# cvxgrp/qcqp

Measured on AMD Instinct MI355X. Metric: restarts x coord-sweeps / sec (improve COORD_DESCENT phase-2 sweeps, 2n^2 flops each; whole step timed), higher is better.
Workload: dtype f64

## Files before the change

### qcqp_amd/csrc/capi_stream.hip

```cpp
#include <chrono>
#include <cstdio>
#include <cstdlib>

#include "capi_ctx.h"
#include "cd_life.h"

using namespace qcqpmi;

namespace {

StreamShape stream_shape(const qcqpmi_ctx *c) {
    StreamShape s;
    s.NB = (int)(c->n16 / 16); s.sep = c->sep; s.maxc = c->maxc; s.Kreal = c->Kreal; s.objclass = c->objclass; s.symcls = c->symcls;
    s.queue_ok = cd_queue_shape_ok(c);
    return s;
}

StreamSwitches stream_switches(const qcqpmi_ctx *c) {
    StreamSwitches s;
    s.life_version = c->life_version; s.force_generic = c->force_generic; s.dbg = c->dbg; s.lr_RB = c->lr_RB; s.profile = c->profile;
    const char *ev = getenv("QCQPMI_L2_PREBUILT");
    s.prebuilt = !(ev && atoi(ev) == 0);
    ev = getenv("QCQPMI_L2_Y0_MAX");
    s.y0_max = ev ? atoll(ev) : STREAM_Y0_ALL;
    ev = getenv("QCQPMI_L2_ROT");
    s.rot = ev ? atoi(ev) : STREAM_ROT_AUTO;
    ev = getenv("QCQPMI_L2_TILES");
    s.tiles = ev ? atoi(ev) : 0;
    return s;
}

int stream_plan_for(qcqpmi_ctx *c, int64_t K, int64_t R, StreamPlan *P) {
    int cus = 0;
    HIPCHK(c, hipDeviceGetAttribute(&cus, hipDeviceAttributeMultiprocessorCount, c->device));
    *P = stream_plan(stream_shape(c), stream_switches(c), K, R, cus);
    return 0;
}

int cd_bestK_reserve(qcqpmi_ctx *c, size_t K) {
    HIPCHK(c, c->d_bestK_idx.reserve(c->stream, K * 2, false));
    HIPCHK(c, c->d_bestK_key.reserve(c->stream, K * 2, false));
    HIPCHK(c, c->d_bestK_x.reserve(c->stream, K * (size_t)c->n, false));
    return 0;
}

int cd_life2_reserve(qcqpmi_ctx *c, size_t scratch) {
    HIPCHK(c, c->l2_scratch.reserve(c->stream, scratch));
    HIPCHK(c, c->l2_abort.reserve(c->stream, 4));
    HIPCHK(c, c->l2_cuslot.reserve(c->stream, 4096));
    if (!c->l2_S) {
        const size_t NB = (size_t)(c->n16 / 16);
        HIPCHK(c, c->l2_D.reserve(c->stream, NB * 256));
        HIPCHK(c, c->l2_S.reserve(c->stream, NB * 48));
        hipError_t e = (hipError_t)cd_life2_pack(c->dp, c->l2_D, c->l2_S, c->stream);
        if (e != hipSuccess) return fail(c, QCQPMI_EHIP, "cd_life2_pack: %s", hipGetErrorString(e));
    }
    return 0;
}

int cd_life2_pre_reserve(qcqpmi_ctx *c, const StreamPlan &P) {
    HIPCHK(c, c->l2_preslack.reserve(c->stream, P.l2_preslack));
    HIPCHK(c, c->l2_y0.reserve(c->stream, P.l2_y0, false));
    return 0;
}

int stream_reserve(qcqpmi_ctx *c, const StreamPlan &P, bool winners) {
    int rc;
    if (P.outputs && (rc = cd_outputs_reserve(c, (int64_t)P.outputs))) return rc;
    if (winners && P.bestK && (rc = cd_bestK_reserve(c, P.bestK))) return rc;
    HIPCHK(c, c->d_qnext.reserve(c->stream, 16));
    HIPCHK(c, c->d_life.reserve(c->stream, 1, false));
    if (P.kernel == STREAM_LIFE2 && (rc = cd_life2_reserve(c, P.l2_scratch))) return rc;
    if (P.pre && (rc = cd_life2_pre_reserve(c, P))) return rc;
    return 0;
}

struct StreamClock {
    const bool on = getenv("QCQPMI_STREAM_TIMING") != nullptr;
    double stage[6] = {0, 0, 0, 0, 0, 0}, step[6] = {0, 0, 0, 0, 0, 0};
    static double now() { return std::chrono::duration<double, std::milli>(std::chrono::steady_clock::now().time_since_epoch()).count(); }
    void at_stage(int k) { stage[k] = now(); }
    void at_step(int k) { step[k] = now(); }
    void report_launch() const {
        if (on) fprintf(stderr, "cd_stream_run launch (ms): reserve %.3f, event %.3f, launch call %.3f, event + spin wait %.3f, copy call %.3f, sync %.3f\n", step[0] - stage[1], step[1] - step[0], step[2] - step[1], step[3] - step[2], step[4] - step[3], step[5] - step[4]);
    }
    void report() const {
        if (on) fprintf(stderr, "cd_stream_run timing (ms): set-up %.3f, launch + kernel %.3f, fetch %.3f, status %.3f, best %.3f\n", stage[1] - stage[0], stage[2] - stage[1],
                        stage[3] - stage[2], stage[4] - stage[3], stage[5] - stage[4]);
    }
};

struct StreamRun {
    int64_t K, R, num_iters;
    double tol;
    uint64_t seed, first_index;
};

int stream_fill_life(qcqpmi_ctx *c, const StreamPlan &P, const StreamRun &r, int generate, int phase1, double viol_tol, uint64_t seed_stride,
                     uint64_t first_stride) {
    HIPCHK(c, hipMemsetAsync(c->d_qnext, 0, 16 * sizeof(int), c->stream));
    CdLife L;
    L.on = 1; L.generate = generate ? 1 : 0; L.phase1 = phase1 ? 1 : 0; L.Rtotal = r.K * r.R; L.Rpop = r.R;
    L.seed = r.seed; L.seed_stride = seed_stride; L.first_index = r.first_index; L.first_stride = first_stride; L.viol_tol = viol_tol;
    L.sweeps1 = c->d_sweeps1; L.status1 = c->d_status1; L.ran2 = c->d_flag;
    L.prof = nullptr;
    L.prebuilt = P.pre ? 1 : 0; L.preslack = P.pre ? (const double *)c->l2_preslack : nullptr;
    L.y0_count = P.y0_count; L.y0 = P.pre ? (const double *)c->l2_y0 : nullptr;
    if (P.life_prof) {
        HIPCHK(c, c->d_life_prof.reserve(c->stream, P.life_prof, false));
        HIPCHK(c, hipMemsetAsync(c->d_life_prof, 0, P.life_prof * sizeof(long long), c->stream));
        L.prof = c->d_life_prof;
    }
    HIPCHK(c, hipMemcpyAsync(c->d_life, &L, sizeof(L), hipMemcpyHostToDevice, c->stream));
    HIPCHK(c, spin_sync(c->stream));
    return 0;
}

int stream_launch_life2(qcqpmi_ctx *c, const StreamPlan &P, const StreamRun &r, StreamClock &clk) {
    CdLife2Args qa;
    qa.P = c->dp; qa.num_iters = r.num_iters; qa.tol = r.tol; qa.life = c->d_life;
    cd_queue_fill_batch(c, qa.b, r.seed, r.first_index);
    qa.b.R = r.K * r.R;
    qa.scratch = c->l2_scratch; qa.Dpack = c->l2_D; qa.Spack = c->l2_S; qa.abort = c->l2_abort; qa.fbound = c->fbound;
    qa.cuslot = P.rot ? (int *)c->l2_cuslot : nullptr; qa.rotmode = P.rot;
    if (qa.cuslot) HIPCHK(c, hipMemsetAsync(c->l2_cuslot, 0, 4096 * sizeof(int), c->stream));
    qa.dbg = (c->dbg & 2048) ? 1 : 0;
    qa.Gpack = P.lr ? (const double *)c->lr_G : nullptr; qa.Upack = P.lr ? (const double *)c->lr_U : nullptr; qa.RB = P.lr ? c->lr_RB : 0;
    qa.nclass = c->Kreal;
    clk.at_step(0);
    (void)hipEventRecord(c->timers[2].beg, c->stream);
    clk.at_step(1);
    hipError_t qe = P.pre ? (hipError_t)cd_life2_prep_launch(c->dp, c->d_life, c->X, r.K * r.R, r.num_iters, r.tol, c->stream) : hipSuccess;
    if (qe == hipSuccess && P.y0_count > 0)
        qe = (hipError_t)cd_life2_y0_launch(c->X, c->lr_U, c->l2_y0, (int)(c->n16 / 16), P.factor_rb, c->n16, P.y0_count, c->stream);
    if (qe == hipSuccess) qe = (hipError_t)cd_life2_launch(qa, P.nmw, P.cs, P.kind, P.tiles, (int)P.wgs, c->stream);
    clk.at_step(2);
    (void)hipEventRecord(c->timers[2].end, c->stream);
    c->timers[2].valid = true;
    if (qe != hipSuccess) return fail(c, QCQPMI_EHIP, "cd_stream_run: %s", hipGetErrorString(qe));
    c->last_cd2_kernel = P.name;
    int ab = 0;
    HIPCHK(c, spin_sync(c->stream));
    clk.at_step(3);
    HIPCHK(c, hipMemcpyAsync(&ab, c->l2_abort, sizeof(int), hipMemcpyDeviceToHost, c->stream));
    clk.at_step(4);
    HIPCHK(c, spin_sync(c->stream));
    clk.at_step(5);
    clk.report_launch();
    if (ab) {
        HIPCHK(c, hipMemsetAsync(c->l2_abort, 0, sizeof(int), c->stream));
        c->R = 0;
        return fail(c, QCQPMI_EHIP, "cd_stream_run: a wait inside cd_life_kernel ran into its watchdog (internal error; no results)");
    }
    return 0;
}

int stream_launch_round4(qcqpmi_ctx *c, const StreamPlan &P, const StreamRun &r) {
    CdQueueArgs qa;
    qa.P = c->dp; qa.num_iters = r.num_iters; qa.tol = r.tol;
    qa.life = c->d_life; qa.life_on = 1;
// ... 134 lines not shown
```

### qcqp_amd/csrc/cd_life.hip

```cpp
#include "cd_life.h"

#include <cstdio>
#include <cstdlib>

#include "onevar.h"
#include "cd_phase1_sep.h"
#include "cd_chain.h"
#include "cd_roles.h"

namespace qcqpmi {
namespace {

constexpr int L2_WD = 1 << 21;
enum { L2_ABORT = 3 };

__device__ __attribute__((always_inline)) inline RqOwn l2_own(int NB, int CS, int m, int NMW) {
    RqOwn o;
    const int rest = NB - CS;
    o.NB = NB;
    if (m < 0) { o.first = rest; o.stride = 1; o.nu = CS; }
    else { o.first = m; o.stride = NMW; o.nu = m < rest ? (rest - m + NMW - 1) / NMW : 0; }
    return o;
}

// ... 11 lines not shown
    int *p1cols = (int *)(smem + 16); \
    int *jn = (int *)(smem + 32); \
    double *sp = smem + L2_SHARED_DOUBLES + (tile_) * l2_tile_doubles(NMW, CSU, LRV, KCLV, MAXC); \
    double *part2 = sp; sp += 2 * NMW * 256; \
    double *fixp = sp; sp += 256; \
    double *gtile = sp; sp += 256; \
    double *DU2 = sp; sp += 2 * 256; \
    double *sc2 = sp; sp += 2 * 48; \
    double *ring = sp; sp += 4 * 256; \
    double *cshare = sp; sp += CSU * 256; \
    double *slk = sp; sp += 16; \
    rq_lds_int *sy = (rq_lds_int *)(int *)sp; sp += 8; \
    double *of0 = sp; sp += 16; \
    long long *ovis = (long long *)sp; sp += 16; \
    long long *oacc = (long long *)sp; sp += 16; \
    long long *oswp = (long long *)sp; sp += 16; \
    int *sid = (int *)sp; sp += 8; \
    int *snew = (int *)sp; sp += 8; \
    int *sfin = (int *)sp; sp += 8; \
    int *ost = (int *)sp; sp += 8; \
    int *gatep = (int *)sp; sp += 8; \
    long long *cst = (long long *)sp; sp += 64 * 10; \
    unsigned long long *sseed = (unsigned long long *)sp; sp += 16; \
    unsigned long long *sfirst = (unsigned long long *)sp; sp += 16; \
    unsigned long long *p1key = (unsigned long long *)sp; sp += 16; \
    int *p1upd = (int *)sp; sp += 8; \
    int *p1fin = (int *)sp; sp += 8; \
    int *p1sw = (int *)sp; sp += 8; \
    int *p1st = (int *)sp; sp += 8; \
    L2Par *par = (L2Par *)sp; sp += 32;       \
    double *ytile = sp; sp += LRV ? L2_YBMAX * 256 : 0; \
    double *pend = sp; sp += LRV ? 2 * 256 : 0; \
    SetTable<MAXC> TC;        \
    TC.slots = 16 * KCLV; \
    TC.lo = sp; sp += (MAXC + 1) * 16 * KCLV; \
    TC.hi = sp; sp += (MAXC + 1) * 16 * KCLV; \
    TC.n = (int *)sp; sp += 8 * KCLV; \
    TC.slow = (int *)sp; sp += 8 * KCLV; \
    int *clsb = (int *)sp;
template <class T>
__device__ __attribute__((always_inline)) inline T *l2_tl(T *p, int t, int tile_doubles) { return (T *)((double *)p + t * tile_doubles); }

struct L2Par {
    const double *Apack, *Apack2, *Dpack, *Spack;
    const double *Gpack, *Upack;
    int RB, pad_;
    double *Xg;
    int *next;
    unsigned long long *prof;
    long long num_iters, n16;
    double tol, r0, fbound;
    int NB, KS, n, nlast, Rtotal, dbg;
    const int *cls;
};
static_assert(sizeof(L2Par) <= 32 * sizeof(double), "L2Par outgrew its LDS slot");
struct L2Life {
    int64_t Rtotal, Rpop, y0_count;
    uint64_t seed, seed_stride, first_index, first_stride;
    const double *preslack, *y0;
    int64_t *sweeps1;
    int *status1;
    uint8_t *ran2;
    unsigned long long *prof;
    double cp, cq, cr;
    int rel, prebuilt;
    int turn, pad_;
};
static_assert(sizeof(L2Life) <= 256, "L2Life outgrew the tail of the LDS allocation");
__device__ __attribute__((always_inline)) inline int l2_uni(int v) { return __builtin_amdgcn_readfirstlane(v); }
__device__ __attribute__((always_inline)) inline long long l2_uni(long long v) {
    const int lo = __builtin_amdgcn_readfirstlane((int)(v & 0xffffffffll)), hi = __builtin_amdgcn_readfirstlane((int)(v >> 32));
    return ((long long)hi << 32) | (long long)(unsigned)lo;
}
__device__ __attribute__((always_inline)) inline double l2_uni(double v) { return __longlong_as_double(l2_uni(__double_as_longlong(v))); }
template <class T>
__device__ __attribute__((always_inline)) inline T *l2_uni(T *p) { return (T *)(uintptr_t)l2_uni((long long)(uintptr_t)p); }

template <int NMW, int CS>
__device__ __attribute__((noinline)) void l2_mfma_role(int m_in, int t_in) {
    constexpr int MAXC = 1;
    constexpr int KCLV = 1;
    constexpr int CSU = CS > 0 ? CS : 1;
    constexpr int LRV = 0;
    const int tile = l2_uni(t_in);
    L2_LDS_VIEW(tile)
    (void)ytile; (void)pend; (void)clsb;
    (void)fixp; (void)gtile; (void)DU2; (void)sc2; (void)cshare; (void)slk; (void)TC; (void)of0; (void)ovis; (void)oacc; (void)oswp; (void)sid; (void)snew;
    (void)sfin; (void)ost; (void)ctl; (void)cst; (void)sseed; (void)sfirst; (void)p1key; (void)p1upd; (void)p1fin; (void)p1sw; (void)p1st; (void)gatep; (void)simdof; (void)p1cols; (void)jn;
    const int lane = threadIdx.x & 63;
    const int m = l2_uni(m_in);
    const double *pApack2 = l2_uni(par->Apack2);
    double *pXg = l2_uni(par->Xg);
    unsigned long long *pprof = l2_uni(par->prof);
    const int NB = l2_uni(par->NB), KS = l2_uni(par->KS);
    const int64_t n16 = l2_uni(par->n16);
    const int rowmask = (l2_uni(par->dbg) & 1) ? 7 : -1;
    const int64_t gmax = (int64_t)1 << 40;
    const RqOwn own = l2_own(NB, CS, m, NMW);
    const int nu = own.nu;
    v2d_ arP[2 * RQ_PFU];
    const unsigned vlane = (unsigned)lane * 16u;
    const __amdgpu_buffer_rsrc_t arsrc = __builtin_amdgcn_make_buffer_rsrc(const_cast<double *>(pApack2), 0, NB * KS * 512, 0x00020000);
    const __amdgpu_buffer_rsrc_t xrsrc = __builtin_amdgcn_make_buffer_rsrc(pXg, 0, (int)(n16 * 128), 0x00020000);
    const int rowstride = KS * 512;
    typedef unsigned rq_u4 __attribute__((ext_vector_type(4)));
    typedef unsigned rq_u2 __attribute__((ext_vector_type(2)));
    #define L2_LDA(dst, soff, vo) { const rq_u4 t0_ = __builtin_amdgcn_raw_buffer_load_b128(arsrc, (vo), (soff), 0);           \
                            const rq_u4 t1_ = __builtin_amdgcn_raw_buffer_load_b128(arsrc, (vo) + 1024u, (soff), 0);   \
                            (dst)[0] = __builtin_bit_cast(v2d_, t0_); (dst)[1] = __builtin_bit_cast(v2d_, t1_); }
    double bq[4 * RQ_PERS];
    {
        const unsigned vl8 = (unsigned)lane * 8u;
    #pragma unroll
        for (int u = 0; u < RQ_PERS; u++)
    #pragma unroll
            for (int q = 0; q < 4; q++) {
                const rq_u2 t_ = __builtin_amdgcn_raw_buffer_load_b64(xrsrc, vl8, (m + NMW * u) * 2048 + q * 512, 0);
                bq[4 * u + q] = __builtin_bit_cast(double, t_);
            }
// ... 184 lines not shown
            for (;;) {
                const rq_i4 s4 = rq_sync_read(sy);
                if (s4[RQ_STOP]) { stop = true; break; }
                if (s4[RQ_CONS] >= (int)i - 1) break;
                if (++spins > L2_WD) { stop = true; rq_sync_write(sy, L2_ABORT, 1, lane); rq_sync_write(sy, RQ_STOP, 1, lane); break; }
                __builtin_amdgcn_s_sleep(1);
            }
            if (stop) break;
            spins = 0;
        }
        {
            double *part = part2 + (int)(i & 1) * NMW * 256 + m * 256;
    #pragma unroll
            for (int v = 0; v < 4; v++) part[v * 64 + (lane & 15) * 4 + (lane >> 4)] = acc[v];
        }
        rq_sync_write(sy, RQ_PARTS + m, (int)i + 1, lane);
        row = row2;
    }
    if (yrow == NB - 1 && iy >= 3) {
        v2d_ aU[YU][2];
    #pragma unroll
        for (int u = 0; u < YU; u++)
            if (u < nu) L2_LDF(aU[u], ursrc, ((NB - 3) * RB + m + NMW * u) * 2048)
        rq_lds_cd *src = rbase + (int)((iy - 2) & 3) * 256;
        double bd[4];
    #pragma unroll
        for (int q = 0; q < 4; q++) bd[q] = src[q * 64];
    #pragma unroll
        for (int v = 0; v < 4; v++)
    #pragma unroll
            for (int u = 0; u < YU; u++)
                if (u < nu) y[u] = __builtin_amdgcn_mfma_f64_16x16x4f64(aU[u][v >> 1][v & 1], bd[v], y[u], 0, 0, 0);
        save_y();
    } else if (yrow == 0) {
        save_y();
    }
    #undef L2_LDF
}

template <int NMW, int CS, int KIND, int TILES, int LR>
__device__ __attribute__((noinline)) void l2_chain_role(int t_in) {
    constexpr bool MULTI = KIND == L2_KIND_GENK || KIND == L2_KIND_LINK;
    constexpr int BK = KIND == L2_KIND_GENK ? L2_KIND_GEN : KIND == L2_KIND_LINK ? L2_KIND_LIN : KIND;
    constexpr int MAXC = MULTI ? 2 : 1;
    constexpr int KCLV = MULTI ? L2_KCL : 1;
    constexpr int CSU = CS > 0 ? CS : 1;
    constexpr int LRV = LR;
    static_assert(!LR || CS == 0, "factored objective: the chain has no share of the contraction");
    static_assert(!MULTI || (TILES == 1 && !LR), "multi-class kinds: one tile per workgroup, no objective factor");
    constexpr bool PRE = BK == L2_KIND_LIN || BK == L2_KIND_SGN;
    const int tile = TILES > 1 ? l2_uni(t_in) : 0;
    L2_LDS_VIEW(tile)
    (void)ytile; (void)pend; (void)clsb;
    (void)slk; (void)snew; (void)p1key; (void)p1upd; (void)p1fin; (void)p1sw; (void)p1st; (void)gatep; (void)simdof; (void)p1cols; (void)jn;
    const int lane = threadIdx.x & 63, r = lane >> 2, gq = lane & 3;
    GLB const double *Apk = glb(l2_uni(par->Apack));
    GLB const double *Apk2 = glb(l2_uni(par->Apack2));
    GLB const double *Dpk = glb(l2_uni(par->Dpack));
    GLB const double *Spk = glb(l2_uni(par->Spack));
    GLB double *Xg = glb(l2_uni(par->Xg));
    GLB const int *pnext = glb(l2_uni(par->next));
    GLB const int *clsg = glb(l2_uni(par->cls));
    unsigned long long *pprof = l2_uni(par->prof);
    const int pRtotal = l2_uni(par->Rtotal);
    const int NB = l2_uni(par->NB), KS = l2_uni(par->KS), nlast = l2_uni(par->nlast);
    struct { int64_t n; double r0; } P = {(int64_t)l2_uni(par->n), l2_uni(par->r0)};
    struct { double tol, fbound; int64_t num_iters; } a = {l2_uni(par->tol), l2_uni(par->fbound), (int64_t)l2_uni(par->num_iters)};
    const int64_t gmax = (int64_t)1 << 40;
    __builtin_amdgcn_s_setprio(3);
    const int Un = TC.n[r], Uslow = TC.slow[r];
    const double Ul0 = TC.lo[r], Uh0 = TC.hi[r], Ul1 = TC.lo[16 + r], Uh1 = TC.hi[16 + r];
    const bool two = Un >= 2;
    const double thr = two ? 1e-7 * (Ul1 - Uh0) : 0.0;
    const double syma = two ? Ul1 : 0.0, symb = two ? Uh1 : Uh0;
    const double gmid = two ? 0.5 * (Uh0 + Ul1) : QM_INF;
    const double linL = Ul0, linH = two ? Uh1 : Uh0;
    auto lin_tl = [&](double l0_, double h0_, double l1_, double h1_, bool two_) {
        const double lL = l0_, lH = two_ ? h1_ : h0_;
        const double w0 = h0_ - l0_, w1 = two_ ? h1_ - l1_ : w0;
        const double wmin = w0 < w1 ? w0 : w1;
        const double hh = fabs(lL) > fabs(lH) ? fabs(lL) : fabs(lH);
        const double scale = a.fbound * (hh * hh > 1.0 ? hh * hh : 1.0);
        return (wmin > 0.0) ? 0.5e-12 * scale / wmin : QM_INF;
    };
    double tl = 0.0;
    if ((BK == L2_KIND_LIN || BK == L2_KIND_SGN) && !MULTI) tl = lin_tl(Ul0, Uh0, Ul1, Uh1, two);
    const double omid = (BK == L2_KIND_SGN) ? 0.5 * (linL + linH) : 0.0;
    struct { int upd_counter, visits, accepted, sweeps, status; bool conv; } S;
    S.upd_counter = (int)cst[0 * 64 + lane]; S.visits = (int)cst[1 * 64 + lane]; S.accepted = (int)cst[2 * 64 + lane];
    S.sweeps = (int)cst[3 * 64 + lane]; S.conv = cst[4 * 64 + lane] != 0; S.status = (int)cst[5 * 64 + lane];
    double fpart = __longlong_as_double(cst[6 * 64 + lane]);
    bool frz = (cst[7 * 64 + lane] & 1) != 0, done = (cst[7 * 64 + lane] & 2) != 0, pre = PRE && (cst[7 * 64 + lane] & 4) != 0;
    bool ld = LR && (cst[7 * 64 + lane] & 8) != 0;
    double facc = __longlong_as_double(cst[8 * 64 + lane]);
    const bool occupied = sid[r] >= 0;
    const RqOwn cown = l2_own(NB, CS, -1, NMW);
    v2d_ arC[2 * CSU];
    double afix[4] = {0.0, 0.0, 0.0, 0.0}, afix2[4] = {0.0, 0.0, 0.0, 0.0};
    v4d_ carry = {0.0, 0.0, 0.0, 0.0};
    double xon[4], d4[4], s3 = 0.0;
    {
    #pragma unroll
        for (int e = 0; e < 4; e++) d4[e] = Dpk[lane + 64 * e];
        if (lane < 48) s3 = Spk[lane];
    #pragma unroll
        for (int v = 0; v < 4; v++) xon[v] = Xg[(4 * v + gq) * 16 + r];
    #pragma unroll
        for (int e = 0; e < 4; e++) DU2[lane + 64 * e] = d4[e];
        if (lane < 48) sc2[lane] = s3;
        if (MULTI && lane < 16) clsb[lane] = (lane < l2_uni(par->n)) ? clsg[lane] : 0;
        v4d_ c0 = {0.0, 0.0, 0.0, 0.0}, c1 = {0.0, 0.0, 0.0, 0.0};
        const int bl2 = NB - 2, bl1 = NB - 1;
        double f0a[4], f0b[4], f1b[4], x2[4], x1[4];
    #pragma unroll
        for (int u = 0; u < 4; u++) {
            f0a[u] = Apk[((int64_t)0 * KS + 4 * bl2 + u) * 64 + lane];
            f0b[u] = Apk[((int64_t)0 * KS + 4 * bl1 + u) * 64 + lane];
            f1b[u] = Apk[((int64_t)1 * KS + 4 * bl1 + u) * 64 + lane];
            x2[u] = LR ? pend[u * 64 + lane] : Xg[(4 * bl2 + u) * 64 + lane];
            x1[u] = LR ? pend[256 + u * 64 + lane] : Xg[(4 * bl1 + u) * 64 + lane];
        }
    #pragma unroll
        for (int u = 0; u < 4; u++) c0 = __builtin_amdgcn_mfma_f64_16x16x4f64(f0a[u], x2[u], c0, 0, 0, 0);
    #pragma unroll
        for (int u = 0; u < 4; u++) {
            c0 = __builtin_amdgcn_mfma_f64_16x16x4f64(f0b[u], x1[u], c0, 0, 0, 0);
            c1 = __builtin_amdgcn_mfma_f64_16x16x4f64(f1b[u], x1[u], c1, 0, 0, 0);
        }
        carry = c1;
        if (CS > 0) {
            rq_load_A<CSU>(arC, Apk2, KS, cown, lane, 0);
            double bqC[4 * CSU];
    #pragma unroll
            for (int U = 0; U < CSU; U++) {
                const int bb = rq_block(cown, U);
    #pragma unroll
                for (int q = 0; q < 4; q++) bqC[4 * U + q] = Xg[(4 * bb + q) * 64 + lane];
            }
    #pragma unroll
            for (int U = 0; U < CSU; U++)
    #pragma unroll
                for (int q = 0; q < 4; q++) cshare[U * 256 + q * 64 + lane] = bqC[4 * U + q];
            c0 = rq_product<CSU>(arC, bqC, Apk2, KS, cown, lane, rq_slot(cown, bl1), rq_slot(cown, bl2), 1, c0);
        }
    #pragma unroll
        for (int v = 0; v < 4; v++) fixp[v * 64 + (lane & 15) * 4 + (lane >> 4)] = c0[v];
    }
    const double tolv = a.tol;
    int b = 0, spins = 0;
    bool wdog = false;
    const bool prof_on = pprof != nullptr;
    long long pw_part = 0, pt_sum = 0, pt_steps = 0, pt_end = 0, pt_fix = 0, pt_req = 0, ptl = 0;
    if (prof_on) { ptl = (long long)__builtin_amdgcn_s_memtime(); if (lane == 0) atomicAdd(pprof + 18, (unsigned long long)(ptl - *(long long *)(ctl + 6))); }
    int pn_int = 0, pn_gen = 0;
#define L2_TICK(acc) if (prof_on) { const long long now_ = (long long)__builtin_amdgcn_s_memtime(); acc += now_ - ptl; ptl = now_; }
    int64_t last_g = 0;
    for (int64_t g = 0; g < gmax; g++) {
        last_g = g;
        const int bn = (b + 1 == NB) ? 0 : b + 1, bn2 = (bn + 1 == NB) ? 0 : bn + 1;
        const int bprev = (b == 0) ? NB - 1 : b - 1;
        const int cur = (int)(g & 1);
        const double *DU = DU2 + cur * 256, *hqb = sc2 + cur * 48, *rtb = sc2 + cur * 48 + 16, *dgb = sc2 + cur * 48 + 32;
        const double *part = part2 + cur * NMW * 256;
        double *rb = ring + (int)(g & 3) * 256;
        const int ncol = (b == NB - 1) ? nlast : 16;
        double xo[4];
    #pragma unroll
        for (int v = 0; v < 4; v++) xo[v] = xon[v];
    #pragma unroll
        for (int e = 0; e < 4; e++) d4[e] = Dpk[(int64_t)bn * 256 + lane + 64 * e];
        if (lane < 48) s3 = Spk[(int64_t)bn * 48 + lane];
        int c3 = 0;
        if (MULTI && lane < 16) c3 = (16 * bn + lane < (int)P.n) ? clsg[16 * bn + lane] : 0;
    #pragma unroll
        for (int v = 0; v < 4; v++) xon[v] = Xg[(16 * (int64_t)bn + 4 * v + gq) * 16 + r];
        {
            GLB const double *ap = Apk + ((int64_t)bn * KS + 4 * b) * 64 + lane;
            GLB const double *ap2 = Apk + ((int64_t)bn2 * KS + 4 * b) * 64 + lane;
    #pragma unroll
            for (int u = 0; u < 4; u++) { afix[u] = ap[u * 64]; afix2[u] = ap2[u * 64]; }
        }
        const long long tw0 = prof_on ? (long long)__builtin_amdgcn_s_memtime() : 0;
        for (;;) {
            const rq_i4 p4 = rq_sync_read(sy + RQ_PARTS);
            int lo4 = p4[0] < p4[1] ? p4[0] : p4[1];
            const int lo2 = p4[2] < p4[3] ? p4[2] : p4[3];
            lo4 = lo4 < lo2 ? lo4 : lo2;
            if (NMW > 4) {
                const rq_i4 q4 = rq_sync_read(sy + RQ_PARTS + 4);
                const int l1 = q4[0] < q4[1] ? q4[0] : q4[1], l2 = q4[2] < q4[3] ? q4[2] : q4[3];
                lo4 = lo4 < l1 ? lo4 : l1;
                lo4 = lo4 < l2 ? lo4 : l2;
            }
            if (lo4 >= (int)g + 1) break;
            if (++spins > L2_WD) { wdog = true; break; }
            __builtin_amdgcn_s_sleep(1);
        }
        if (wdog) { rq_sync_write(sy, L2_ABORT, 1, lane); break; }
        spins = 0;
        if (prof_on) { pt_req += tw0 - ptl; ptl = (long long)__builtin_amdgcn_s_memtime(); pw_part += ptl - tw0; pn_int++; }
        double gb[4], xn[4], rto[4], t2o[4], hq4[4];
    #pragma unroll
        for (int v = 0; v < 4; v++) {
            double s = fixp[v * 64 + lane];
    #pragma unroll
            for (int w = 0; w < NMW; w++) s += part[w * 256 + v * 64 + lane];
            hq4[v] = hqb[4 * v + gq];
            s += hq4[v];
            gb[v] = s;
            gtile[(4 * v + gq) * 16 + r] = s;
        }
        rq_sync_write(sy, RQ_CONS, (int)g + 1, lane);
    #pragma unroll
        for (int v = 0; v < 4; v++) { rto[v] = rtb[4 * v + gq]; t2o[v] = dgb[4 * v + gq]; }
        if (b == 0 && !S.conv && S.sweeps >= (int)a.num_iters) {
            S.conv = true;
            frz = true; facc = 0.0;
        }
        if (b == 0 && !S.conv) S.sweeps++;
        const bool act = !S.conv;
        int nv[4], slv[4];
        double l0v[4], h0v[4], l1v[4], h1v[4], midv[4], thrv[4], tlv[4], tolev[4];
    #pragma unroll
        for (int v = 0; v < 4; v++) {
            if (MULTI) {
                const int s_ = clsb[cur * 16 + 4 * v + gq] * 16 + r;
                nv[v] = TC.n[s_]; slv[v] = TC.slow[s_];
                l0v[v] = TC.lo[s_]; h0v[v] = TC.hi[s_]; l1v[v] = TC.lo[16 * KCLV + s_]; h1v[v] = TC.hi[16 * KCLV + s_];
// ... 349 lines not shown
            const unsigned hw = __builtin_amdgcn_s_getreg(4 | (0 << 6) | (31 << 11)), xcc = __builtin_amdgcn_s_getreg(20 | (0 << 6) | (31 << 11));
            arrival = glb_add(glb(a0.cuslot) + (((xcc & 15) << 8) | (((hw >> 12) & 15) << 4) | ((hw >> 8) & 15)), 1);
        }
        simdof[8] = (arrival & 1) ? (a0.rotmode == 2 ? 16 + 1 : 2) : 0;
    }
    if (tid0 < 64 * TILES) {
        long long *cs_ = l2_tl(cst, tid0 >> 6, TD);
#pragma unroll
        for (int f = 0; f < 10; f++) cs_[f * 64 + (tid0 & 63)] = (f == 4) ? 1 : 0;
    }
    if (tid0 < NS) { l2_tl(sid, tid0 >> 4, TD)[tid0 & 15] = -1; l2_tl(sfin, tid0 >> 4, TD)[tid0 & 15] = 0; }
    GLB const CdLife *lf0 = glb(a0.life);
    const long long life_t0 = (tid0 == 0 && lf0->prof) ? (long long)__builtin_amdgcn_s_memtime() : 0;
    __syncthreads();
    int role, rtile = 0;
    {
        int cnt[4] = {0, 0, 0, 0};
        int rank = 0;
        const int mys = simdof[wave];
#pragma unroll
        for (int w = 0; w < NW; w++) {
            const int s = simdof[w];
#pragma unroll
            for (int q = 0; q < 4; q++) cnt[q] += (s == q) ? 1 : 0;
            rank += (s == mys && w < wave) ? 1 : 0;
        }
        const bool even = cnt[0] == NW / 4 && cnt[1] == NW / 4 && cnt[2] == NW / 4 && cnt[3] == NW / 4;
        if (NMW == 3 && TILES == 1) {
            const int rot = simdof[8];
            if (!even) role = wave;
            else if (rot >= 16) role = mys == 0 ? 0 : 1 + ((mys - 1 + (rot - 16)) % 3);
            else role = (mys + rot) & 3;
        }
        else if (TILES == 2) { role = even ? mys : (wave & 3); rtile = even ? rank : (wave >> 2); }
        else if (even) role = (mys == 0) ? (rank == 0 ? 0 : 7) : mys + 3 * rank;
        else role = wave;
        role = __builtin_amdgcn_readfirstlane(role);
        rtile = __builtin_amdgcn_readfirstlane(rtile);
        if (tid0 == 0 && lf0->prof) {
            if (even) atomicAdd((unsigned long long *)lf0->prof + 6, 1ull);
            const unsigned hw = __builtin_amdgcn_s_getreg(4 | (0 << 6) | (31 << 11)), xcc = __builtin_amdgcn_s_getreg(20 | (0 << 6) | (31 << 11));
            Xg0[0] = (double)(((xcc & 15) << 8) | (((hw >> 13) & 7) << 4) | ((hw >> 8) & 15));
        }
    }
    const int nlast = (int)(P.n - 16 * (int64_t)(NB - 1));
    if (tid0 < TILES) {
        L2Par *pr = l2_tl(par, tid0, TD);
        pr->Apack = P.Apack; pr->Apack2 = P.Apack2; pr->Dpack = a0.Dpack; pr->Spack = a0.Spack;
        pr->Gpack = a0.Gpack; pr->Upack = a0.Upack; pr->RB = a0.RB; pr->pad_ = 0;
        pr->Xg = a0.scratch + ((int64_t)blockIdx.x * TILES + tid0) * n16 * 16; pr->next = a0.b.next; pr->prof = (unsigned long long *)lf0->prof;
        pr->num_iters = a.num_iters; pr->n16 = n16; pr->tol = a.tol; pr->r0 = P.r0; pr->fbound = a.fbound;
        pr->NB = NB; pr->KS = KS; pr->n = (int)P.n; pr->nlast = nlast; pr->Rtotal = (int)lf0->Rtotal; pr->dbg = a0.dbg;
        pr->cls = P.cls;
    }
    L2Life *const lfl = (L2Life *)(smem + L2_SHARED_DOUBLES + TILES * TD);
    (void)lfl;
    if constexpr (LR != 0) {
        if (tid0 == 0) {
            lfl->Rtotal = lf0->Rtotal; lfl->Rpop = lf0->Rpop; lfl->y0_count = lf0->y0_count;
            lfl->seed = lf0->seed; lfl->seed_stride = lf0->seed_stride; lfl->first_index = lf0->first_index; lfl->first_stride = lf0->first_stride;
            lfl->preslack = lf0->preslack; lfl->y0 = lf0->y0; lfl->sweeps1 = lf0->sweeps1; lfl->status1 = lf0->status1; lfl->ran2 = lf0->ran2;
            lfl->prof = (unsigned long long *)lf0->prof; lfl->prebuilt = lf0->prebuilt;
            const int e0 = P.cptr[P.krep[0]];
            lfl->cp = P.cp[e0]; lfl->cq = P.cq[e0]; lfl->cr = P.cr[e0]; lfl->rel = P.crel[e0];
            lfl->turn = (lf0->prebuilt && lf0->Rtotal > (int64_t)gridDim.x * NS) ? 1 : 0; lfl->pad_ = 0;
        }
    }
    __syncthreads();

    for (;;) {
        int tid = tid0;
        asm volatile("" : "+v"(tid));
        const CdLife *lifep = a0.life;
        asm volatile("" : "+s"(lifep));
        const int lane = tid & 63, r = lane >> 2;
        bool turned = false;
        if constexpr (LR != 0) {
            if (l2_uni(lfl->turn)) {
                turned = true;
                __builtin_amdgcn_s_setprio(3);
                unsigned long long *const profp = l2_uni(lfl->prof);
                const long long pt0 = profp ? (long long)__builtin_amdgcn_s_memtime() : 0;
                const int r16 = 16 * a0.RB;
                const int y0n = (int)l2_uni((long long)lfl->y0_count);
                int oldid = -1, idv = -1, nwv = 0, nnew = 0;
                double nslack = 0.0;
                long long nsw1 = 0;
                int nst1 = 0, nran2 = 0;
                if (tid < NS) {
                    const int st = tid >> 4, sc = tid & 15;
                    int id = l2_tl(sid, st, TD)[sc];
                    if (l2_tl(sfin, st, TD)[sc]) {
                        oldid = id; id = -1;
                        glb(a0.b.visits)[oldid] = l2_tl(ovis, st, TD)[sc]; glb(a0.b.accepted)[oldid] = l2_tl(oacc, st, TD)[sc]; glb(a0.b.sweeps)[oldid] = l2_tl(oswp, st, TD)[sc];
                        glb(a0.b.status)[oldid] = l2_tl(ost, st, TD)[sc];
                        if (a0.b.f0out) glb(a0.b.f0out)[oldid] = l2_tl(of0, st, TD)[sc];
                        glb(lfl->sweeps1)[oldid] = l2_tl(p1sw, st, TD)[sc]; glb(lfl->status1)[oldid] = l2_tl(p1st, st, TD)[sc];
                        glb(lfl->ran2)[oldid] = (uint8_t)l2_tl(gatep, st, TD)[sc];
                        l2_tl(sfin, st, TD)[sc] = 0;
                    }
                    if (id < 0) {
                        const int idx = glb_add(glb(a0.b.next), 1);
                        if (idx < (int)lfl->Rtotal) {
                            id = idx; nwv = 1;
                            nslack = glb(lfl->preslack)[idx]; nsw1 = glb(lfl->sweeps1)[idx]; nst1 = glb(lfl->status1)[idx]; nran2 = glb(lfl->ran2)[idx];
                            const uint64_t pop = (uint64_t)idx / (uint64_t)lfl->Rpop, rho = (uint64_t)idx % (uint64_t)lfl->Rpop;
                            l2_tl(sseed, st, TD)[sc] = lfl->seed + pop * lfl->seed_stride;
                            l2_tl(sfirst, st, TD)[sc] = lfl->first_index + pop * lfl->first_stride + rho - (uint64_t)idx;
                        }
                    }
                    idv = id;
                    l2_tl(sid, st, TD)[sc] = id; l2_tl(snew, st, TD)[sc] = nwv; l2_tl(p1upd, st, TD)[sc] = oldid;
                    l2_tl(p1key, st, TD)[sc] = ordered_key(-QM_INF);
                    *(volatile rq_lds_int *)(l2_tl((int *)sy, st, TD) + sc) = (sc >= RQ_PARTS + NMW) ? 0x7fffffff : 0;
                    const unsigned long long mturn = __builtin_amdgcn_ballot_w64(oldid >= 0 || nwv || id < 0);
                    const unsigned long long mocc = __builtin_amdgcn_ballot_w64(id >= 0), mnew = __builtin_amdgcn_ballot_w64(nwv != 0);
                    if (oldid >= 0 || nwv || id < 0) p1cols[__builtin_popcountll(mturn & ((1ull << tid) - 1ull))] = tid;
                    nnew = __builtin_popcountll(mnew);
                    if (tid == 0) { ctl[0] = __builtin_popcountll(mocc); ctl[4] = __builtin_popcountll(mturn); jn[0] = 0; jn[1] = 0; }
                }
                __syncthreads();
                {
                    const double cp = l2_uni(lfl->cp), cq = l2_uni(lfl->cq), cr = l2_uni(lfl->cr);
                    const int rel = l2_uni(lfl->rel);
                    GLB const double *y0g = glb(l2_uni(lfl->y0));
                    const int nturn = l2_uni(ctl[4]);
                    const int KR = (int)((n16 + NT - 1) / NT), KI = KR + (r16 + NT - 1) / NT;
                    const int np = (int)P.n, nx = (int)n16;
                    constexpr int L2_TCH = 16;
                    double vacc = -QM_INF;
                    int ci0 = 0, k0 = 0;
                    while (ci0 < nturn) {
                        double xo[L2_TCH], xn[L2_TCH];
                        int ci = ci0, k = k0;
#pragma unroll
                        for (int q = 0; q < L2_TCH; q++) {
                            xo[q] = 0.0; xn[q] = 0.0;
                            if (ci < nturn) {
                                const int c = l2_uni(p1cols[ci]), ct = c >> 4, cc = c & 15;
                                const int oid = l2_uni(l2_tl(p1upd, ct, TD)[cc]), id = l2_uni(l2_tl(sid, ct, TD)[cc]), nw = l2_uni(l2_tl(snew, ct, TD)[cc]);
                                if (k < KR) {
                                    const int j = k * NT + tid;
                                    if (oid >= 0 && j < np) xo[q] = (Xg0 + (int64_t)ct * n16 * 16)[(int64_t)j * 16 + cc];
                                    if (nw && j < nx) xn[q] = glb(a0.b.X)[((int64_t)(id >> 4) * n16 + j) * 16 + (id & 15)];
                                } else {
                                    const int row = (k - KR) * NT + tid;
                                    if (nw && id < y0n && row < r16) xn[q] = y0g[((int64_t)(id >> 4) * r16 + row) * 16 + (id & 15)];
                                }
                                if (++k == KI) { k = 0; ci++; }
                            }
                        }
                        ci = ci0; k = k0;
#pragma unroll
                        for (int q = 0; q < L2_TCH; q++) {
                            if (ci < nturn) {
                                const int c = l2_uni(p1cols[ci]), ct = c >> 4, cc = c & 15;
                                const int oid = l2_uni(l2_tl(p1upd, ct, TD)[cc]), id = l2_uni(l2_tl(sid, ct, TD)[cc]), nw = l2_uni(l2_tl(snew, ct, TD)[cc]);
                                if (k < KR) {
                                    const int j = k * NT + tid;
                                    if (oid >= 0) {
                                        if (j < nx) glb(a0.b.X)[((int64_t)(oid >> 4) * n16 + j) * 16 + (oid & 15)] = xo[q];
                                        if (j < np) {
                                            const double f = (cp * xo[q] + cq) * xo[q] + cr;
                                            const double vv = (rel == RELOP_EQ) ? fabs(f) : (f > 0.0 ? f : 0.0);
                                            vacc = vv > vacc ? vv : vacc;
                                        }
                                        if (k == KR - 1) {
                                            const double vw = wave_max(vacc);
                                            if (lane == 0) atomicMax(&l2_tl(p1key, ct, TD)[cc], ordered_key(vw));
                                            vacc = -QM_INF;
                                        }
                                    }
                                    if ((nw || id < 0) && j < nx) {
                                        (Xg0 + (int64_t)ct * n16 * 16)[(int64_t)j * 16 + cc] = xn[q];
                                        if (j >= nx - 32) l2_tl(pend, ct, TD)[(j - (nx - 32)) * 16 + cc] = (nw && id < y0n) ? xn[q] : 0.0;
                                    }
                                } else {
                                    const int row = (k - KR) * NT + tid;
                                    if ((nw || id < 0) && row < r16) l2_tl(ytile, ct, TD)[row * 16 + cc] = xn[q];
                                }
                                if (++k == KI) { k = 0; ci++; }
                            }
                        }
                        ci0 = ci; k0 = k;
                    }
                }
                if (tid < NS && (nwv || idv < 0)) {
                    const int st = tid >> 4, sc = tid & 15;
                    if (nwv) { l2_tl(p1fin, st, TD)[sc] = 0; l2_tl(p1sw, st, TD)[sc] = (int)nsw1; l2_tl(p1st, st, TD)[sc] = nst1; l2_tl(gatep, st, TD)[sc] = nran2; }
                    l2_tl(slk, st, TD)[sc] = nslack;
                    L2_STORE_SETS(st, sc, nslack)
                }
                __syncthreads();
                if (tid < NS && oldid >= 0 && a0.b.mvout) glb(a0.b.mvout)[oldid] = ordered_unkey(l2_tl(p1key, tid >> 4, TD)[tid & 15]);
                if (ctl[0] == 0) break;
                if (nlast < 16) {
                    for (int w = tid; w < NS * (16 - nlast); w += NT) {
                        const int c = w % NS, ct = c >> 4, cc = c & 15, row = w / NS;
                        const int id = l2_tl(sid, ct, TD)[cc];
                        if (l2_tl(snew, ct, TD)[cc] || id < 0) {
                            const int nn = l2_tl(TC.n, ct, TD)[cc];
                            double xp = 0.0;
                            static_assert(BK == L2_KIND_BAND || BK == L2_KIND_GEN, "turnover pass: padding fixed point of the band and gen kinds only");
                            if (BK == L2_KIND_BAND) xp = nn >= 2 ? l2_tl(TC.lo, ct, TD)[16 * KCLV + cc] : 0.0;
                            else xp = nn >= 1 ? l2_tl(TC.hi, ct, TD)[cc] : 0.0;
                            if (!(xp == xp) || __builtin_isinf(xp)) xp = 0.0;
                            (Xg0 + (int64_t)ct * n16 * 16)[(P.n + row) * 16 + cc] = xp;
                            l2_tl(pend, ct, TD)[(16 + nlast + row) * 16 + cc] = (id >= 0 && id < y0n) ? xp : 0.0;
                        }
                    }
                }
                if (profp && tid == 0) {
                    atomicAdd(profp + 0, (unsigned long long)((long long)__builtin_amdgcn_s_memtime() - pt0));
                    atomicAdd(profp + 2, 1ull);
                    atomicAdd(profp + 3, (unsigned long long)nnew);
                }
                __builtin_amdgcn_s_setprio(0);
            }
        }
        if (!turned) {
            if (tid == 0) { ctl[0] = 0; jn[0] = 0; jn[1] = 0; }
            __syncthreads();
            if (tid < NS) {
                const int st = tid >> 4, sc = tid & 15;
                int id = l2_tl(sid, st, TD)[sc], nw = 0;
                if (id < 0) {
                    GLB const CdLife *lf = glb(lifep);
                    const int idx = glb_add(glb(a0.b.next), 1);
                    if (idx < (int)lf->Rtotal) {
                        id = idx; nw = 1;
                        const uint64_t pop = (uint64_t)idx / (uint64_t)lf->Rpop, rho = (uint64_t)idx % (uint64_t)lf->Rpop;
                        l2_tl(sseed, st, TD)[sc] = lf->seed + pop * lf->seed_stride;
                        l2_tl(sfirst, st, TD)[sc] = lf->first_index + pop * lf->first_stride + rho - (uint64_t)idx;
                    }
// ... 630 lines not shown
```

### qcqp_amd/csrc/cd_life_plan.h

```cpp
#pragma once
#include <stddef.h>
#include <stdint.h>

namespace qcqpmi {

constexpr int RQ_NSIMD = 3;
constexpr int RQ_MAXU = 20;
constexpr int RQ_CSMAX = 6;
constexpr int L2_YBMAX = 18;
constexpr int L2_KCL = 4;

enum { L2_KIND_BAND = 0, L2_KIND_GEN = 1, L2_KIND_LIN = 2, L2_KIND_GENK = 3, L2_KIND_LINK = 4, L2_KIND_SGN = 5 };

inline int chain_share(int NB, int dbg) {
    int cs = (dbg & 128) ? ((dbg >> 8) & 7) : 4;
    cs = cs > RQ_CSMAX ? RQ_CSMAX : cs;
    if (cs >= NB) cs = 0;
    cs &= ~1;
    return cs;
}

inline bool chain_range_ok(int NB, int cs) { return NB - cs <= RQ_NSIMD * RQ_MAXU && NB >= 3; }

inline bool cd_life2_factor_ok(int NB, int64_t r) {
// ... 15 lines not shown
    else if (NB - 4 <= 3 * RQ_MAXU) { w = 3; c = (NB < 8) ? 2 : 4; }
    else if (factor_rb > 0 && !multi && objclass == 1 && NB <= 256) { w = 3; c = 0; }
    else if (NB - 4 <= 7 * RQ_MAXU) { w = 7; c = 4; }
    else return false;
    *nmw = w; *cs = c;
    *kind = objclass == 0 ? L2_KIND_SGN : multi ? (objclass == 2 ? L2_KIND_LINK : L2_KIND_GENK) : objclass == 2 ? L2_KIND_LIN : (symcls ? L2_KIND_BAND : L2_KIND_GEN);
    return true;
}

inline int cd_life2_tiles(int nmw, int cs, int requested, int lr) {
    if (!lr || nmw != 3 || cs != 0) return 1;
    return requested == 2 ? 2 : 1;
}

inline const char *cd_life2_name(int nmw, int kind, int tiles, int lr) {
    if (kind == L2_KIND_GENK) return nmw == 3 ? "cd_life_kernel<3,gen,classes>" : "cd_life_kernel<7,gen,classes>";
    if (kind == L2_KIND_LINK) return nmw == 3 ? "cd_life_kernel<3,lin,classes>" : "cd_life_kernel<7,lin,classes>";
    if (kind == L2_KIND_SGN) return nmw == 3 ? "cd_life_kernel<3,sgn>" : "cd_life_kernel<7,sgn>";
    if (lr) return tiles == 2 ? (kind == L2_KIND_BAND ? "cd_life_kernel<3,band,2 tiles,factored>" : "cd_life_kernel<3,gen,2 tiles,factored>")
                              : (kind == L2_KIND_BAND ? "cd_life_kernel<3,band,factored>" : "cd_life_kernel<3,gen,factored>");
    if (tiles == 2) return kind == L2_KIND_BAND ? "cd_life_kernel<3,band,2 tiles>" : kind == L2_KIND_GEN ? "cd_life_kernel<3,gen,2 tiles>" : "cd_life_kernel<3,lin,2 tiles>";
    if (nmw == 3) return kind == L2_KIND_BAND ? "cd_life_kernel<3,band>" : kind == L2_KIND_GEN ? "cd_life_kernel<3,gen>" : "cd_life_kernel<3,lin>";
    return kind == L2_KIND_BAND ? "cd_life_kernel<7,band>" : kind == L2_KIND_GEN ? "cd_life_kernel<7,gen>" : "cd_life_kernel<7,lin>";
}

constexpr int64_t L2_Y0_BUDGET = (int64_t)2 << 30;
constexpr long long STREAM_Y0_ALL = 0x7fffffffffffffffLL;
inline int64_t cd_life2_y0_count(int64_t KR, int RB, long long y0_max) {
    int64_t cnt = KR;
    { const long long m = y0_max; cnt = m < 0 ? 0 : (m < cnt ? m : cnt); }
    const int64_t fit = L2_Y0_BUDGET / ((int64_t)RB * 16 * 16 * (int64_t)sizeof(double)) * 16;
    return cnt < fit ? cnt : fit;
}

struct StreamShape {
    int NB;
    bool sep;
    int maxc, Kreal, objclass;
    bool symcls;
    bool queue_ok;
};

constexpr int STREAM_ROT_AUTO = -0x7fffffff - 1;
struct StreamSwitches {
    int life_version;
    bool force_generic;
    int dbg;
    int lr_RB;
    bool profile;
    bool prebuilt;
    long long y0_max;
    int rot;
    int tiles;
};

enum { STREAM_NONE = 0, STREAM_LIFE2 = 1, STREAM_ROUND4 = 2 };

struct StreamPlan {
    bool supported;
    bool range_only;
    int kernel;
    int nmw, cs, kind;
    bool lr;
    int factor_rb;
    bool pre;
    int tiles;
    int64_t wgs;
    int64_t y0_count;
    int rot;
    const char *name;
    size_t l2_scratch, l2_preslack, l2_y0, life_prof;
    size_t outputs;
    size_t bestK;
};

inline StreamPlan stream_plan(const StreamShape &sh, const StreamSwitches &sw, int64_t K, int64_t R, int cus) {
    StreamPlan p = StreamPlan();
    p.name = "";
    const int NB = sh.NB;
    int nmw = 0, cs2 = 0, kind = 0;
    const int factor_rb = (sw.lr_RB > 0 && sw.life_version != 3 && cd_life2_factor_ok(NB, 16 * (int64_t)sw.lr_RB)) ? sw.lr_RB : 0;
    const bool use2 = sw.life_version != 1 && !sw.force_generic && !(sw.dbg & 64) && sh.sep &&
                      cd_life2_config(NB, sh.sep, sh.maxc, sh.Kreal, sh.objclass, sh.symcls, factor_rb, &nmw, &cs2, &kind);
    if (!use2) {
        const bool eligible = !sw.force_generic && !(sw.dbg & 64) && sh.queue_ok && NB - 4 <= RQ_NSIMD * RQ_MAXU && NB >= 3;
        if (!eligible || sw.life_version != 1) return p;
        const int cs = chain_share(NB, sw.dbg);
        if (!chain_range_ok(NB, cs)) { p.range_only = true; return p; }
        p.supported = true; p.kernel = STREAM_ROUND4; p.cs = cs;
        p.wgs = (K * R + 15) / 16 < cus ? (K * R + 15) / 16 : cus;
        p.name = "cd_phase2_qs_kernel<lifecycle>";
    } else {
        const bool lr = factor_rb > 0 && nmw == 3 && (kind == L2_KIND_BAND || kind == L2_KIND_GEN);
        if (lr) cs2 = 0;
        if (!lr && (sw.dbg & 128)) { const int k2 = (sw.dbg >> 8) & 7; if (nmw == 3 && (k2 == 0 || k2 == 2 || k2 == 4) && k2 < NB) cs2 = k2; }
        p.supported = true; p.kernel = STREAM_LIFE2; p.nmw = nmw; p.cs = cs2; p.kind = kind; p.lr = lr; p.factor_rb = factor_rb;
        p.pre = lr && sw.prebuilt;
        p.y0_count = p.pre ? cd_life2_y0_count(K * R, factor_rb, sw.y0_max) : 0;
        p.tiles = cd_life2_tiles(nmw, cs2, sw.tiles, lr ? 1 : 0);
        p.wgs = (K * R + 16 * p.tiles - 1) / (16 * p.tiles);
        const int maxw = cd_life2_max_wgs(nmw, cus, p.tiles);
        if (p.wgs > maxw) p.wgs = maxw;
        if (sw.dbg & 1024) { const int lim = (sw.dbg >> 12) & 1023; if (lim > 0 && p.wgs > lim) p.wgs = lim; }
        p.rot = sw.rot != STREAM_ROT_AUTO ? sw.rot : (lr ? 2 : 0);
        p.name = cd_life2_name(nmw, kind, p.tiles, lr ? 1 : 0);
        p.l2_scratch = (size_t)cd_life2_max_wgs(nmw, cus, 1) * (size_t)NB * 256;
        if (p.pre) {
            p.l2_preslack = (size_t)(K * R);
            p.l2_y0 = (size_t)((p.y0_count + 15) / 16) * (size_t)factor_rb * 256;
        }
    }
    p.life_prof = sw.profile ? 24 : 0;
    p.outputs = (size_t)(K * R);
    p.bestK = (size_t)K;
    return p;
}

}
```

### qcqp_amd/csrc/cd_queue.h

```cpp
#pragma once
#include <hip/hip_runtime.h>
#include <stdint.h>
#include "kernels.h"

namespace qcqpmi {

struct CdBatch {
    double *X;
    const double *f0cur;
    const double *slack;
    const uint8_t *flag;
    int64_t *visits, *accepted, *sweeps;
    int *status;
    double *f0out, *mvout;
    int64_t R;
    uint64_t seed, first_index;
    int *next;
};

struct CdLife {
    int on;
    int generate;
    int phase1;
    int64_t Rtotal, Rpop;
    uint64_t seed, seed_stride, first_index, first_stride;
    double viol_tol;
    int64_t *sweeps1;
    int *status1;
    uint8_t *ran2;
    long long *prof;
    int prebuilt;
    const double *preslack;
    int64_t y0_count;
    const double *y0;
};

struct CdQueueArgs {
    DevProblem P;
    CdBatch b;
    int64_t num_iters;
    double tol;
    const CdLife *life;
    int life_on;
};

size_t cd_queue_lds_bytes(const DevProblem &P);
int cd_queue_launch(const CdQueueArgs &a, int cs, int max_wgs, hipStream_t st);

}
```

Measured before the change: 30.28 million.

## Lazily read fresh restart x from population buffer instead of copying into tile

When a slot takes a new prebuilt restart, the turnover loop now copies only the head and tail of its x vector into the per-tile buffer instead of the whole vector. The chain role in the low-rank kernel reads x for new slots directly from the global population buffer through a per-slot base pointer. The aim is to cut global-memory copy traffic during restart turnover. In exchange it adds per-slot pointer selection to the hot x load and couples correctness to when the snew flag is set.

```diff
diff --git a/qcqp_amd/csrc/capi_stream.hip b/qcqp_amd/csrc/capi_stream.hip
--- a/qcqp_amd/csrc/capi_stream.hip
+++ b/qcqp_amd/csrc/capi_stream.hip
@@ -27,6 +27,8 @@
     s.rot = ev ? atoi(ev) : STREAM_ROT_AUTO;
     ev = getenv("QCQPMI_L2_TILES");
     s.tiles = ev ? atoi(ev) : 0;
+    ev = getenv("QCQPMI_L2_LAZYX");
+    s.lazyx = !(ev && atoi(ev) == 0);
     return s;
 }
 
@@ -106,6 +108,7 @@
     L.prof = nullptr;
     L.prebuilt = P.pre ? 1 : 0; L.preslack = P.pre ? (const double *)c->l2_preslack : nullptr;
     L.y0_count = P.y0_count; L.y0 = P.pre ? (const double *)c->l2_y0 : nullptr;
+    L.lazyx = P.lazyx ? 1 : 0;
     if (P.life_prof) {
         HIPCHK(c, c->d_life_prof.reserve(c->stream, P.life_prof, false));
         HIPCHK(c, hipMemsetAsync(c->d_life_prof, 0, P.life_prof * sizeof(long long), c->stream));
diff --git a/qcqp_amd/csrc/cd_life.hip b/qcqp_amd/csrc/cd_life.hip
--- a/qcqp_amd/csrc/cd_life.hip
+++ b/qcqp_amd/csrc/cd_life.hip
@@ -87,6 +87,7 @@
     double tol, r0, fbound;
     int NB, KS, n, nlast, Rtotal, dbg;
     const int *cls;
+    const double *Xpop;
 };
 static_assert(sizeof(L2Par) <= 32 * sizeof(double), "L2Par outgrew its LDS slot");
 struct L2Life {
@@ -99,7 +100,7 @@
     unsigned long long *prof;
     double cp, cq, cr;
     int rel, prebuilt;
-    int turn, pad_;
+    int turn, lazy;
 };
 static_assert(sizeof(L2Life) <= 256, "L2Life outgrew the tail of the LDS allocation");
 __device__ __attribute__((always_inline)) inline int l2_uni(int v) { return __builtin_amdgcn_readfirstlane(v); }
@@ -390,7 +391,7 @@
     const int tile = TILES > 1 ? l2_uni(t_in) : 0;
     L2_LDS_VIEW(tile)
     (void)ytile; (void)pend; (void)clsb;
-    (void)slk; (void)snew; (void)p1key; (void)p1upd; (void)p1fin; (void)p1sw; (void)p1st; (void)gatep; (void)simdof; (void)p1cols; (void)jn;
+    (void)slk; (void)p1key; (void)p1upd; (void)p1fin; (void)p1sw; (void)p1st; (void)gatep; (void)simdof; (void)p1cols; (void)jn;
     const int lane = threadIdx.x & 63, r = lane >> 2, gq = lane & 3;
     GLB const double *Apk = glb(l2_uni(par->Apack));
     GLB const double *Apk2 = glb(l2_uni(par->Apack2));
@@ -432,6 +433,15 @@
     bool ld = LR && (cst[7 * 64 + lane] & 8) != 0;
     double facc = __longlong_as_double(cst[8 * 64 + lane]);
     const bool occupied = sid[r] >= 0;
+    auto x_base = [&](int ro) -> GLB const double * {
+        GLB const double *p = Xg + ro;
+        const double *xpop = l2_uni(par->Xpop);
+        const int id = sid[ro];
+        if (xpop != nullptr && snew[ro] != 0 && id >= 0) p = glb(xpop) + ((int64_t)(id >> 4) * (int64_t)NB * 16) * 16 + (id & 15);
+        return p;
+    };
+    (void)x_base;
+    if (LR == 0) { (void)snew; }
     const RqOwn cown = l2_own(NB, CS, -1, NMW);
     v2d_ arC[2 * CSU];
     double afix[4] = {0.0, 0.0, 0.0, 0.0}, afix2[4] = {0.0, 0.0, 0.0, 0.0};
@@ -510,8 +520,18 @@
         if (lane < 48) s3 = Spk[(int64_t)bn * 48 + lane];
         int c3 = 0;
         if (MULTI && lane < 16) c3 = (16 * bn + lane < (int)P.n) ? clsg[16 * bn + lane] : 0;
-    #pragma unroll
-        for (int v = 0; v < 4; v++) xon[v] = Xg[(16 * (int64_t)bn + 4 * v + gq) * 16 + r];
+        int ro = r;
+        GLB const double *xs = Xg;
+        if constexpr (LR != 0) {
+            asm volatile("" : "+v"(ro));
+            xs = (g < NB - 3) ? x_base(ro) : Xg + ro;
+        }
+        (void)xs; (void)ro;
+    #pragma unroll
+        for (int v = 0; v < 4; v++) {
+            if constexpr (LR != 0) xon[v] = xs[(16 * (int64_t)bn + 4 * v + gq) * 16];
+            else xon[v] = Xg[(16 * (int64_t)bn + 4 * v + gq) * 16 + r];
+        }
         {
             GLB const double *ap = Apk + ((int64_t)bn * KS + 4 * b) * 64 + lane;
             GLB const double *ap2 = Apk + ((int64_t)bn2 * KS + 4 * b) * 64 + lane;
@@ -967,6 +987,7 @@
         pr->num_iters = a.num_iters; pr->n16 = n16; pr->tol = a.tol; pr->r0 = P.r0; pr->fbound = a.fbound;
         pr->NB = NB; pr->KS = KS; pr->n = (int)P.n; pr->nlast = nlast; pr->Rtotal = (int)lf0->Rtotal; pr->dbg = a0.dbg;
         pr->cls = P.cls;
+        if constexpr (LR != 0) pr->Xpop = (lf0->prebuilt && lf0->lazyx && lf0->Rtotal > (int64_t)gridDim.x * NS) ? a0.b.X : nullptr;
     }
     L2Life *const lfl = (L2Life *)(smem + L2_SHARED_DOUBLES + TILES * TD);
     (void)lfl;
@@ -978,7 +999,8 @@
             lfl->prof = (unsigned long long *)lf0->prof; lfl->prebuilt = lf0->prebuilt;
             const int e0 = P.cptr[P.krep[0]];
             lfl->cp = P.cp[e0]; lfl->cq = P.cq[e0]; lfl->cr = P.cr[e0]; lfl->rel = P.crel[e0];
-            lfl->turn = (lf0->prebuilt && lf0->Rtotal > (int64_t)gridDim.x * NS) ? 1 : 0; lfl->pad_ = 0;
+            lfl->turn = (lf0->prebuilt && lf0->Rtotal > (int64_t)gridDim.x * NS) ? 1 : 0;
+            lfl->lazy = (lfl->turn && lf0->lazyx) ? 1 : 0;
         }
     }
     __syncthreads();
@@ -1040,8 +1062,9 @@
                     const int rel = l2_uni(lfl->rel);
                     GLB const double *y0g = glb(l2_uni(lfl->y0));
                     const int nturn = l2_uni(ctl[4]);
-                    const int KR = (int)((n16 + NT - 1) / NT), KI = KR + (r16 + NT - 1) / NT;
+                    const int KR = (int)((n16 + NT - 1) / NT), KY = (r16 + NT - 1) / NT;
                     const int np = (int)P.n, nx = (int)n16;
+                    const int lz = l2_uni(lfl->lazy);
                     constexpr int L2_TCH = 16;
                     double vacc = -QM_INF;
                     int ci0 = 0, k0 = 0;
@@ -1054,15 +1077,17 @@
                             if (ci < nturn) {
                                 const int c = l2_uni(p1cols[ci]), ct = c >> 4, cc = c & 15;
                                 const int oid = l2_uni(l2_tl(p1upd, ct, TD)[cc]), id = l2_uni(l2_tl(sid, ct, TD)[cc]), nw = l2_uni(l2_tl(snew, ct, TD)[cc]);
-                                if (k < KR) {
-                                    const int j = k * NT + tid;
+                                const bool tail = lz && oid < 0 && id >= 0;
+                                const int kx = tail ? 1 : KR;
+                                if (k < kx) {
+                                    const int j = tail ? (tid < 16 ? tid : nx - 48 + tid) : k * NT + tid;
                                     if (oid >= 0 && j < np) xo[q] = (Xg0 + (int64_t)ct * n16 * 16)[(int64_t)j * 16 + cc];
-                                    if (nw && j < nx) xn[q] = glb(a0.b.X)[((int64_t)(id >> 4) * n16 + j) * 16 + (id & 15)];
+                                    if (nw && j < nx && (!lz || j < 16 || j >= nx - 32)) xn[q] = glb(a0.b.X)[((int64_t)(id >> 4) * n16 + j) * 16 + (id & 15)];
                                 } else {
-                                    const int row = (k - KR) * NT + tid;
+                                    const int row = (k - kx) * NT + tid;
                                     if (nw && id < y0n && row < r16) xn[q] = y0g[((int64_t)(id >> 4) * r16 + row) * 16 + (id & 15)];
                                 }
-                                if (++k == KI) { k = 0; ci++; }
+                                if (++k == kx + KY) { k = 0; ci++; }
                             }
                         }
                         ci = ci0; k = k0;
@@ -1071,8 +1096,10 @@
                             if (ci < nturn) {
                                 const int c = l2_uni(p1cols[ci]), ct = c >> 4, cc = c & 15;
                                 const int oid = l2_uni(l2_tl(p1upd, ct, TD)[cc]), id = l2_uni(l2_tl(sid, ct, TD)[cc]), nw = l2_uni(l2_tl(snew, ct, TD)[cc]);
-                                if (k < KR) {
-                                    const int j = k * NT + tid;
+                                const bool tail = lz && oid < 0 && id >= 0;
+                                const int kx = tail ? 1 : KR;
+                                if (k < kx) {
+                                    const int j = tail ? (tid < 16 ? tid : nx - 48 + tid) : k * NT + tid;
                                     if (oid >= 0) {
                                         if (j < nx) glb(a0.b.X)[((int64_t)(oid >> 4) * n16 + j) * 16 + (oid & 15)] = xo[q];
                                         if (j < np) {
@@ -1086,15 +1113,15 @@
                                             vacc = -QM_INF;
                                         }
                                     }
-                                    if ((nw || id < 0) && j < nx) {
+                                    if ((nw || id < 0) && j < nx && (!lz || !nw || j < 16 || j >= nx - 32)) {
                                         (Xg0 + (int64_t)ct * n16 * 16)[(int64_t)j * 16 + cc] = xn[q];
                                         if (j >= nx - 32) l2_tl(pend, ct, TD)[(j - (nx - 32)) * 16 + cc] = (nw && id < y0n) ? xn[q] : 0.0;
                                     }
                                 } else {
-                                    const int row = (k - KR) * NT + tid;
+                                    const int row = (k - kx) * NT + tid;
                                     if ((nw || id < 0) && row < r16) l2_tl(ytile, ct, TD)[row * 16 + cc] = xn[q];
                                 }
-                                if (++k == KI) { k = 0; ci++; }
+                                if (++k == kx + KY) { k = 0; ci++; }
                             }
                         }
                         ci0 = ci; k0 = k;
diff --git a/qcqp_amd/csrc/cd_life_plan.h b/qcqp_amd/csrc/cd_life_plan.h
--- a/qcqp_amd/csrc/cd_life_plan.h
+++ b/qcqp_amd/csrc/cd_life_plan.h
@@ -91,6 +91,7 @@
     long long y0_max;
     int rot;
     int tiles;
+    bool lazyx = true;
 };
 
 enum { STREAM_NONE = 0, STREAM_LIFE2 = 1, STREAM_ROUND4 = 2 };
@@ -103,6 +104,7 @@
     bool lr;
     int factor_rb;
     bool pre;
+    bool lazyx;
     int tiles;
     int64_t wgs;
     int64_t y0_count;
@@ -135,6 +137,7 @@
         if (!lr && (sw.dbg & 128)) { const int k2 = (sw.dbg >> 8) & 7; if (nmw == 3 && (k2 == 0 || k2 == 2 || k2 == 4) && k2 < NB) cs2 = k2; }
         p.supported = true; p.kernel = STREAM_LIFE2; p.nmw = nmw; p.cs = cs2; p.kind = kind; p.lr = lr; p.factor_rb = factor_rb;
         p.pre = lr && sw.prebuilt;
+        p.lazyx = p.pre && sw.lazyx;
         p.y0_count = p.pre ? cd_life2_y0_count(K * R, factor_rb, sw.y0_max) : 0;
         p.tiles = cd_life2_tiles(nmw, cs2, sw.tiles, lr ? 1 : 0);
         p.wgs = (K * R + 16 * p.tiles - 1) / (16 * p.tiles);
diff --git a/qcqp_amd/csrc/cd_queue.h b/qcqp_amd/csrc/cd_queue.h
--- a/qcqp_amd/csrc/cd_queue.h
+++ b/qcqp_amd/csrc/cd_queue.h
@@ -33,6 +33,7 @@
     const double *preslack;
     int64_t y0_count;
     const double *y0;
+    int lazyx;
 };
 
 struct CdQueueArgs {
```

Measured after the change: 30.69 million (median of 6 runs). 1.01x the previous value.
